# szpiech/garlic

Measured on AMD Instinct MI355X. Metric: LOD-windows/sec (SNPs x inds / winsize), higher is better.
Workload: dtype f64

## Files before the change

garlic_amd/csrc/garlic_hip.hip:

```cpp
#include "../../include/garlic_hip.h"
#include "lod_kernels.hpp"
#include "variant_kernels.hpp"
#include "ld_kernels.hpp"
#include "tgls_ring_kernel.hpp"
#include "wlod_strip_kernel.hpp"
#include "wlod_small_kernel.hpp"
#include "coverage_kernel.hpp"
#include "roh_segments_kernel.hpp"
#include "feed_kernel.hpp"

#include <algorithm>
#include <chrono>
#include <functional>
#include <mutex>
#include <queue>
#include <cmath>
#include <cstdarg>
#include <cstdio>
#include <cstdlib>
#include <cstring>
#include <string>
#include <thread>
#include <unordered_map>
#include <vector>
// ... 1083 lines not shown
    const bool wlod_small = W < WLOD_R;
    if (wlod_shape_ok && use_gl && (rc = ensure_gl_terms(p, true, M, mu))) return rc;
    const bool wlod_gl = wlod_shape_ok && use_gl && p->glterms_valid && p->glterms_scaled;
    bool wlod_fast = (wlod_shape_ok && !use_gl) || wlod_gl;
    if (wlod_fast && !wlod_gl && sizeof(double) * (size_t)(W + TILE) * 4 + 16 > 150 * 1024) wlod_fast = false;
    if (wlod_fast && !wlod_gl && (rc = ensure_score_rows(p, error, M, mu, W))) return rc;
    if (mode == MODE_WLOD && !wlod_fast && (rc = ensure_rld(p))) return rc;
    const bool wlod_stream = wlod_fast && wlod_small && !p->cov_pending.bits && !getenv("GARLIC_WLOD_SMALL_TILES");
    if (p->cov_pending.bits && mode == MODE_WLOD && !wlod_fast) return GARLIC_INTERNAL_NO_BITS;
    if (wlod_stream && (rc = ensure_rld(p))) return rc;
    if (mode == MODE_WLOD && use_gl && p->gl_cont && !wlod_fast && (rc = ensure_gl_terms(p))) return rc;
    const size_t wlod_rows = wlod_gl ? 0 : sizeof(double) * (size_t)(W + TILE) * 4;
    const size_t wlod_patch = sizeof(double) * (size_t)WAVE * WT_PITCH;
    const bool wlod_use_patch = wlod_rows + 16 + wlod_patch <= 160 * 1024 / 8 && !getenv("GARLIC_WLOD_NO_PATCH");
    const bool wlod_gl_ring = wlod_gl && !wlod_small && (ind_begin & (WAVE - 1)) == 0 && !getenv("GARLIC_WLOD_GL_NO_RING");
    const bool ring_patch = !getenv("GARLIC_WLOD_GL_NO_PATCH");
    const int strip_waves = (W + 15 - 16 * WS_WAVES <= 16 || getenv("GARLIC_WLOD_STRIP_NARROW_ONLY")) ? WS_WAVES : WS_WAVES_WIDE;
    const bool wlod_gl_strip = wlod_gl_ring && W + 15 - 16 * strip_waves <= 16 && !getenv("GARLIC_WLOD_GL_NO_STRIP");
    const bool strip_now = wlod_gl_strip;
    const size_t wlod_lds = wlod_gl_ring ? WLOD_GL_RING_OFF + (size_t)WLOD_WAVES * GARLIC_WLOD_GL_RING_ROWS * WAVE * 8
                                   : wlod_rows + 16 + (wlod_use_patch ? wlod_patch : 0);

    const Layout Lhost = make_layout(p, pitch_align, ind_count);
    const int32_t pitch_align_host = pitch_align;
    if (where == GARLIC_HOST) pitch_align = std::max(pitch_align, 32);
    Layout L = make_layout(p, pitch_align, ind_count, thin_step);
    for (int c = 0; c < p->nchr; c++)
        if (3 * L.pitch[c] * 8 + 512 >= (int64_t)1 << 32)
            return fail(GARLIC_ERR_INVALID, "chromosome %d too long for 32-bit row offsets", c);

    const bool feed_kernel = thin_step > 0;
    uint64_t blocks_hash = 0;
    if (blocks) {
        blocks_hash = 0xCBF29CE484222325ull;
        for (uint8_t b : *blocks) blocks_hash = (blocks_hash ^ (b ? 1u : 2u)) * 0x100000001B3ull;
        blocks_hash |= 1;
    }
    const bool reuse = p->plan.valid && p->plan.blocks_hash == blocks_hash && p->plan.mode == (int)mode && p->plan.W == W &&
                       p->plan.max_gap == max_gap && p->plan.ind_begin == ind_begin &&
                       p->plan.ind_count == ind_count && p->plan.pitch_align == pitch_align &&
                       p->plan.wlod_fast == wlod_fast && p->plan.thin_step == thin_step && p->plan.wlod_strip == wlod_gl_strip &&
                       p->plan.feed_kernel == feed_kernel;
    const int nblk = (ind_count + WAVE - 1) / WAVE;
    std::vector<Run> runs;
    std::vector<FillItem> fill;
    std::vector<ChainItem> items;
    std::vector<FeedItem> feed_items;
    std::vector<ChrDev> chrs;
    int64_t n_valid = p->plan.n_valid;
    size_t n_items = p->plan.n_items, n_fill = p->plan.n_fill, n_feed_items = p->plan.n_feed_items;
    int64_t n_runs = p->plan.n_runs;
    if (!reuse) {
        plan_runs(p, W, runs, fill, n_valid);
        std::vector<int> order(runs.size());
        for (size_t i = 0; i < runs.size(); i++) order[i] = (int)i;
        std::stable_sort(order.begin(), order.end(), [&](int x, int y) {
            return (runs[x].b - runs[x].a) > (runs[y].b - runs[y].a);
        });
        items.reserve(runs.size() * nblk);
        for (size_t i = 0; i < order.size(); i++) {
            const Run &r = runs[order[i]];
            for (int k = 0; k < nblk; k++)
                if (!blocks || (*blocks)[(size_t)k]) items.push_back(ChainItem{r.chr, r.a, r.b, k * WAVE});
        }
        if (feed_kernel) {
            std::vector<int32_t> col0(runs.size());
            for (size_t i = 0; i < runs.size(); i++) {
                const int32_t s = (runs[i].a + thin_step - 1) / thin_step;
                col0[i] = (int64_t)s * thin_step <= runs[i].b ? s : -1;
            }
            build_feed_items(runs, order, blocks, nblk, col0, feed_items);
            n_feed_items = feed_items.size();
            if ((rc = p->d_feed_items.reserve(std::max<size_t>(n_feed_items, 1)))) return rc;
        }
        chrs.resize(p->nchr);
        for (int c = 0; c < p->nchr; c++)
            chrs[c] = ChrDev{p->chr_off[c], L.base[c], L.pitch[c], p->chr_nloci[c],
                             (pitch_align >= 2 && 64 * L.pitch[c] * 8 + 512 < ((int64_t)1 << 32)) ? 1 : 0};
        n_items = items.size();
        n_fill = fill.size();
        n_runs = (int64_t)runs.size();
        if ((rc = p->d_chrs.reserve(chrs.size()))) return rc;
        if ((rc = p->d_items.reserve(std::max<size_t>(n_items, 1)))) return rc;
        if ((rc = p->d_fill.reserve(std::max<size_t>(n_fill, 1)))) return rc;
        if (!p->d_counter.p) {
            if ((rc = p->d_counter.reserve(8))) return rc;
            HIP_TRY(hipMemsetAsync(p->d_counter.p, 0, 8 * sizeof(int32_t), ctx->stream));
        }
        p->plan.valid = false;
    }
    std::vector<uint8_t> valid;
    std::vector<int2> tiles, segs;
    if (wlod_fast && !reuse) {
        valid.assign((size_t)p->nloci, 0);
        for (const Run &r : runs)
            memset(valid.data() + p->chr_off[r.chr] + r.a, 1, (size_t)(r.b - r.a + 1));
        for (int c = 0; c < p->nchr; c++)
            for (int s0 = 0; s0 < p->chr_nloci[c]; s0 += TILE) tiles.push_back(make_int2(c, s0));
        p->plan.n_tiles = (int32_t)tiles.size();
        for (int c = 0; c < p->nchr; c++)
            for (int s0 = 0; s0 < p->chr_nloci[c]; s0 += WSM_T) segs.push_back(make_int2(c, s0));
        p->plan.n_segs = (int32_t)segs.size();
        if ((rc = p->d_valid.reserve(valid.size()))) return rc;
        if ((rc = p->d_tiles.reserve(tiles.size())) || (rc = p->d_segs.reserve(segs.size()))) return rc;
    }
    std::vector<WlodStrip> strips;
    if (wlod_gl_strip && !reuse) {
        int64_t total_groups = 0;
        for (int c = 0; c < p->nchr; c++) total_groups += (p->chr_nloci[c] + WLOD_R - 1) / WLOD_R;
        const int64_t pairs = (nblk + 1) / 2;
        int64_t per = total_groups * pairs / 8192;
        per = std::min<int64_t>(256, std::max<int64_t>(64, per)) & ~(int64_t)1;
        if (const char *e = getenv("GARLIC_WLOD_STRIP_GROUPS")) per = std::max<int64_t>(1, atol(e));
        for (int c = 0; c < p->nchr; c++) {
            const int ng = (p->chr_nloci[c] + WLOD_R - 1) / WLOD_R;
            for (int g0 = 0; g0 < ng; g0 += (int)per)
                strips.push_back(WlodStrip{c, g0 * WLOD_R, std::min<int>((int)per, ng - g0), 0});
        }
        p->plan.n_strips = (int32_t)strips.size();
        if ((rc = p->d_strips.reserve(strips.size()))) return rc;
    }
    int workers = ctx->n_cu;
    if (const char *e = getenv("GARLIC_WORKERS")) workers = std::max(1, atoi(e));
    workers = std::min<int>(workers, (int)n_items);

    double *d_out = out;
    if (where == GARLIC_HOST) {
        if (p->d_out.cap < (size_t)L.total && mode == MODE_LOD && thin_step == 0 && !p->placing &&
            (size_t)L.total * sizeof(double) >= ((size_t)1 << 30) && !getenv("GARLIC_NO_PLACEMENT")) {
            p->placing = true;
            void *best = nullptr;
            rc = garlic_panel_alloc_scores(p, pitch_align, ind_count, W, error, max_gap, 0, &best, nullptr);
            p->placing = false;
            if (rc) return rc;
            p->d_out.adopt(ctx, best, (size_t)L.total);
            return launch_lod(p, mode, W, error, max_gap, M, mu, ind_begin, ind_count, pitch_align_host, out, where, thin_step, blocks);
        }
        if ((rc = p->d_out.reserve(ctx, (size_t)L.total))) return rc;
        d_out = p->d_out.p;
    }
    const bool aligned16 = (pitch_align % 2 == 0) && ((reinterpret_cast<uintptr_t>(d_out) & 15) == 0);

    auto enqueue = [&]() -> int {
    HIP_TRY(hipEventRecord(ctx->ev_begin, ctx->stream));
    if (!reuse) {
        HIP_TRY(hipMemcpyAsync(p->d_chrs.p, chrs.data(), sizeof(ChrDev) * chrs.size(),
                               hipMemcpyHostToDevice, ctx->stream));
        if (n_items)
            HIP_TRY(hipMemcpyAsync(p->d_items.p, items.data(), sizeof(ChainItem) * n_items,
                                   hipMemcpyHostToDevice, ctx->stream));
        if (feed_kernel && n_feed_items)
            HIP_TRY(hipMemcpyAsync(p->d_feed_items.p, feed_items.data(), sizeof(FeedItem) * n_feed_items,
                                   hipMemcpyHostToDevice, ctx->stream));
        if (n_fill)
            HIP_TRY(hipMemcpyAsync(p->d_fill.p, fill.data(), sizeof(FillItem) * n_fill,
                                   hipMemcpyHostToDevice, ctx->stream));
        if (wlod_fast) {
            HIP_TRY(hipMemcpyAsync(p->d_valid.p, valid.data(), valid.size(), hipMemcpyHostToDevice,
                                   ctx->stream));
            HIP_TRY(hipMemcpyAsync(p->d_tiles.p, tiles.data(), sizeof(int2) * tiles.size(),
                                   hipMemcpyHostToDevice, ctx->stream));
            HIP_TRY(hipMemcpyAsync(p->d_segs.p, segs.data(), sizeof(int2) * segs.size(),
                                   hipMemcpyHostToDevice, ctx->stream));
            if (!strips.empty())
                HIP_TRY(hipMemcpyAsync(p->d_strips.p, strips.data(), sizeof(WlodStrip) * strips.size(),
                                       hipMemcpyHostToDevice, ctx->stream));
        }
    }
    if (thin_step > 0) {
        hipLaunchKernelGGL(fill_value_kernel, dim3(1024), dim3(256), 0, ctx->stream, d_out, L.total, MISSING_D);
    } else if (n_fill && !wlod_fast && !cov_bits) {
        dim3 grid((unsigned)n_fill, (unsigned)((ind_count + FILL_ROWS - 1) / FILL_ROWS));
        hipLaunchKernelGGL(fill_missing_kernel, grid, dim3(256), 0, ctx->stream, p->d_fill.p,
                           p->d_chrs.p, ind_count, d_out);
    }
    if (n_items && (!reuse || mode != MODE_LOD)) HIP_TRY(hipMemsetAsync(p->d_counter.p, 0, 2 * sizeof(int32_t), ctx->stream));
    p->stats_slot = (int)(ctx->n_calls % garlic_ctx::HIST);
    HIP_TRY(hipEventRecord(ctx->hist0[p->stats_slot], ctx->stream));
    if (wlod_fast) {
        const bool two_blocks = !wlod_gl && !wlod_small && !getenv("GARLIC_WLOD_ONE_BLOCK");
        const int per_wg = two_blocks ? WLOD2_BLOCKS : WLOD_WAVES;
        const int nquad = (nblk + per_wg - 1) / per_wg;
        WlodArgs a{p->d_valid.p, p->d_chrs.p, p->d_tiles.p, p->nwordrows, p->nchr, ind_begin, ind_count, W, nquad,
                   (uint32_t)((int64_t)p->plan.n_tiles * nquad), ((wlod_gl_ring ? ring_patch : wlod_use_patch) ? 1 : 0) | (getenv("GARLIC_WLOD_NO_PF") ? 2 : 0),
                   (int64_t)(GOFF + p->nloci + GPAD_BACK), wlod_gl_ring ? 1 : 0, p->cov_pending, nullptr, nullptr};
        const uint32_t *a_packed = p->d_packed.p;
        const double *a_wtab = wlod_gl ? p->d_glterms.p : p->d_wtab.p, *a_skew = p->d_skew.p + SKEW_FRONT;
        const unsigned wl_grid = (a.n_work + 7u) / 8u * 8u;
        const dim3 wl_block(WLOD_WAVES * WAVE);
        if (wlod_lds > 48 * 1024 && two_blocks) {
            const void *fn = aligned16 ? (const void *)wlod_tile2_kernel<WLOD_R, true> : (const void *)wlod_tile2_kernel<WLOD_R, false>;
            HIP_TRY(hipFuncSetAttribute(fn, hipFuncAttributeMaxDynamicSharedMemorySize, (int)wlod_lds));
        } else if (wlod_lds > 48 * 1024) {
            const void *fn = wlod_gl ? (aligned16 ? (const void *)wlod_tile_gl_kernel<WLOD_R, true>
                                                  : (const void *)wlod_tile_gl_kernel<WLOD_R, false>)
                                     : (aligned16 ? (const void *)wlod_tile_kernel<WLOD_R, true>
                                                  : (const void *)wlod_tile_kernel<WLOD_R, false>);
            HIP_TRY(hipFuncSetAttribute(fn, hipFuncAttributeMaxDynamicSharedMemorySize, (int)wlod_lds));
        }
        if (wlod_stream && aligned16) {
            const int nquad8 = (nblk + WLOD2_BLOCKS - 1) / WLOD2_BLOCKS;
            WlodArgs as = a;
            as.tiles = p->d_segs.p;
            as.nquad = nquad8;
            as.n_work = (uint32_t)((int64_t)p->plan.n_segs * nquad8);
            as.use_patch = 1;
            const void *fn = wlod_gl ? wlod_stream_small_gl_fn(W) : wlod_stream_small_fn(W);
            const size_t lds = wlod_small_lds_bytes(W);
            if (lds > 48 * 1024) HIP_TRY(hipFuncSetAttribute(fn, hipFuncAttributeMaxDynamicSharedMemorySize, (int)lds));
            const double *a_rld = p->d_rld.p;
            void *kargs[] = {(void *)&a_packed, (void *)&a_wtab, (void *)&a_rld, (void *)&d_out, (void *)&as};
            HIP_TRY(hipLaunchKernel(fn, dim3((as.n_work + 7u) / 8u * 8u), wl_block, kargs, lds, ctx->stream));
        } else if (wlod_small) {
            const void *fn = wlod_gl ? (aligned16 ? (const void *)wlod_tile_small_gl_kernel<WLOD_R, true>
                                                  : (const void *)wlod_tile_small_gl_kernel<WLOD_R, false>)
                                     : (aligned16 ? (const void *)wlod_tile_small_kernel<WLOD_R, true>
                                                  : (const void *)wlod_tile_small_kernel<WLOD_R, false>);
            void *kargs[] = {(void *)&a_packed, (void *)&a_wtab, (void *)&a_skew, (void *)&d_out, (void *)&a};
            HIP_TRY(hipLaunchKernel(fn, dim3(wl_grid), wl_block, kargs, wlod_lds, ctx->stream));
        } else if (strip_now) {
            const int n_pairs = (nblk + 1) / 2;
            WlodStripArgs sa{p->d_valid.p, p->d_chrs.p, p->d_strips.p, p->d_glterms.p, a_skew, d_out,
                             (int64_t)(GOFF + p->nloci + GPAD_BACK), ind_begin, ind_count, W, strip_waves, n_pairs,
                             ring_patch ? 1 : 0, (uint32_t)((int64_t)p->plan.n_strips * n_pairs), p->d_counter.p + 3, p->cov_pending};
// ... 2 lines not shown
            const bool wide = strip_waves == WS_WAVES_WIDE;
            bool three = !wide && aligned16 && !sa.cov.bits && !getenv("GARLIC_WLOD_STRIP_TWO_PER_CU");
            for (int k = 0; three && k < p->nchr; k++) three = L.pitch[k] * 8 < ((int64_t)1 << 32);
            const void *fn = three ? (const void *)wlod_strip_gl3_kernel
                             : wide ? (aligned16 ? (const void *)wlod_strip_gl_kernel<true, WS_WAVES_WIDE>
                                                 : (const void *)wlod_strip_gl_kernel<false, WS_WAVES_WIDE>)
                                    : (aligned16 ? (const void *)wlod_strip_gl_kernel<true, WS_WAVES>
                                                 : (const void *)wlod_strip_gl_kernel<false, WS_WAVES>);
            const uint32_t strip_lds = three ? WF_LDS_BYTES : WS_LDS_BYTES;
            HIP_TRY(hipFuncSetAttribute(fn, hipFuncAttributeMaxDynamicSharedMemorySize, (int)strip_lds));
            void *kargs[] = {(void *)&sa};
            HIP_TRY(hipLaunchKernel(fn, dim3(grid), dim3((strip_waves + 1) * WAVE), kargs, strip_lds, ctx->stream));
            if (getenv("GARLIC_WLOD_STRIP_FORCE_RERUN")) HIP_TRY(hipMemsetAsync(p->d_counter.p + 3, 1, sizeof(int32_t), ctx->stream));
            WlodArgs ar = a;
            ar.run_if = p->d_counter.p + 3;
            ar.rerun_count = p->d_counter.p + 4;
            if (aligned16)
                hipLaunchKernelGGL((wlod_tile_glring_kernel<WLOD_R, true>), dim3(wl_grid), wl_block, wlod_lds, ctx->stream,
                                   a_packed, a_wtab, a_skew, d_out, ar);
            else
                hipLaunchKernelGGL((wlod_tile_glring_kernel<WLOD_R, false>), dim3(wl_grid), wl_block, wlod_lds, ctx->stream,
                                   a_packed, a_wtab, a_skew, d_out, ar);
        } else if (wlod_gl_ring && aligned16)
            hipLaunchKernelGGL((wlod_tile_glring_kernel<WLOD_R, true>), dim3(wl_grid), wl_block, wlod_lds, ctx->stream,
                               a_packed, a_wtab, a_skew, d_out, a);
        else if (wlod_gl_ring)
            hipLaunchKernelGGL((wlod_tile_glring_kernel<WLOD_R, false>), dim3(wl_grid), wl_block, wlod_lds, ctx->stream,
                               a_packed, a_wtab, a_skew, d_out, a);
        else if (wlod_gl && aligned16)
            hipLaunchKernelGGL((wlod_tile_gl_kernel<WLOD_R, true>), dim3(wl_grid), wl_block, wlod_lds, ctx->stream,
                               a_packed, a_wtab, a_skew, d_out, a);
        else if (wlod_gl)
            hipLaunchKernelGGL((wlod_tile_gl_kernel<WLOD_R, false>), dim3(wl_grid), wl_block, wlod_lds, ctx->stream,
                               a_packed, a_wtab, a_skew, d_out, a);
        else if (two_blocks && aligned16)
            hipLaunchKernelGGL((wlod_tile2_kernel<WLOD_R, true>), dim3(wl_grid), wl_block, wlod_lds, ctx->stream,
                               a_packed, a_wtab, a_skew, d_out, a);
        else if (two_blocks)
            hipLaunchKernelGGL((wlod_tile2_kernel<WLOD_R, false>), dim3(wl_grid), wl_block, wlod_lds, ctx->stream,
                               a_packed, a_wtab, a_skew, d_out, a);
        else if (aligned16)
            hipLaunchKernelGGL((wlod_tile_kernel<WLOD_R, true>), dim3(wl_grid), wl_block, wlod_lds, ctx->stream,
                               a_packed, a_wtab, a_skew, d_out, a);
        else
            hipLaunchKernelGGL((wlod_tile_kernel<WLOD_R, false>), dim3(wl_grid), wl_block, wlod_lds, ctx->stream,
                               a_packed, a_wtab, a_skew, d_out, a);
    } else if (n_items && exact) {
        VariantArgs a{p->d_packed.p, p->d_tab.p,  p->d_tabgl.p, p->d_codes.p, p->d_decay.p, p->d_rld.p,
                      p->d_items.p,  p->d_chrs.p, d_out,        p->nind_pad,  p->nwordrows, ind_begin,    ind_count,
                      W,             (int32_t)p->gl_values.size(), use_gl ? 1 : 0,
                      (use_gl && p->gl_cont) ? p->d_glterms.p : nullptr, (int64_t)(GOFF + p->nloci + GPAD_BACK)};
        hipLaunchKernelGGL(lod_chain_exact_kernel, dim3((unsigned)n_items), dim3(WAVE), 0, ctx->stream, a, (int)n_items);
    } else if (n_items && mode == MODE_LOD) {
        ChainArgs a{p->d_packed.p, p->d_tab.p, p->d_items.p,     p->d_chrs.p,     d_out, p->nind_pad, p->nwordrows,
                    ind_begin,     ind_count,  W,               (int32_t)n_items, p->d_counter.p, nullptr};
        DevBuf<int64_t> d_trace;
        const char *trace_path = getenv("GARLIC_TRACE");
        if (trace_path && !(feed_kernel && n_feed_items) && d_trace.reserve(4 * n_items) == GARLIC_OK) {
            (void)hipMemsetAsync(d_trace.p, 0, sizeof(int64_t) * 4 * n_items, ctx->stream);
            a.trace = d_trace.p;
        }
        if (feed_kernel && n_feed_items) {
            FeedArgs f{p->d_packed.p, p->d_tab.p, p->d_feed_items.p, p->d_chrs.p, d_out, nullptr, p->nwordrows, ind_begin, ind_count, W,
                       (int32_t)n_feed_items, thin_step, getenv("GARLIC_FEED_NO_ASM") ? 0 : 1, p->d_counter.p, nullptr};
            DevBuf<int64_t> d_ftrace;
            const char *ftrace_path = getenv("GARLIC_TRACE");
            if (ftrace_path && d_ftrace.reserve(8 * n_feed_items) == GARLIC_OK) {
                (void)hipMemsetAsync(d_ftrace.p, 0, sizeof(int64_t) * 8 * n_feed_items, ctx->stream);
                f.trace = d_ftrace.p;
            }
            const void *fn = (const void *)lod_feed_kernel;
            int grid = (int)std::min<size_t>(n_feed_items, (size_t)ctx->n_cu * std::max(1, p->plan.feed_per_cu));
            if (!reuse && (rc = feed_grid(ctx, feed_items, &grid, &p->plan.feed_per_cu))) return rc;
            void *kargs[] = {(void *)&f};
            HIP_TRY(hipLaunchKernel(fn, dim3((unsigned)grid), dim3(FEED_G * WAVE), kargs, 0, ctx->stream));
            if (f.trace) {
                std::vector<int64_t> tr(8 * n_feed_items);
                (void)hipMemcpyAsync(tr.data(), d_ftrace.p, sizeof(int64_t) * tr.size(), hipMemcpyDeviceToHost, ctx->stream);
                (void)hipStreamSynchronize(ctx->stream);
                if (FILE *fo = fopen(ftrace_path, "w")) {
                    for (size_t i = 0; i < n_feed_items; i++) {
                        fprintf(fo, "%zu", i);
                        for (int q = 0; q < 8; q++) fprintf(fo, " %lld", (long long)tr[8 * i + q]);
                        fprintf(fo, "\n");
                    }
                    fclose(fo);
                }
                d_ftrace.release();
            }
        } else if (aligned16)
            hipLaunchKernelGGL((lod_chain_kernel<true>), dim3((unsigned)workers), dim3(CHAIN_THREADS), 0,
                               ctx->stream, a);
        else
            hipLaunchKernelGGL((lod_chain_kernel<false>), dim3((unsigned)workers), dim3(CHAIN_THREADS), 0,
                               ctx->stream, a);
        if (a.trace) {
            std::vector<int64_t> tr(4 * n_items);
            (void)hipMemcpyAsync(tr.data(), d_trace.p, sizeof(int64_t) * tr.size(), hipMemcpyDeviceToHost, ctx->stream);
            (void)hipStreamSynchronize(ctx->stream);
            if (FILE *f = fopen(trace_path, "w")) {
                for (size_t i = 0; i < n_items; i++)
                    fprintf(f, "%zu %lld %lld %lld %lld %d\n", i, (long long)tr[4 * i], (long long)tr[4 * i + 1],
                            (long long)tr[4 * i + 2], (long long)tr[4 * i + 3], 0);
                fclose(f);
            }
            d_trace.release();
        }
    } else if (n_items) {
        VariantArgs a{p->d_packed.p, p->d_tab.p,  p->d_tabgl.p, p->d_codes.p, p->d_decay.p, p->d_rld.p,
                      p->d_items.p,  p->d_chrs.p, d_out,        p->nind_pad,  p->nwordrows, ind_begin,    ind_count,
                      W,             (int32_t)p->gl_values.size(), use_gl ? 1 : 0,
                      (use_gl && p->gl_cont) ? p->d_glterms.p : nullptr, (int64_t)(GOFF + p->nloci + GPAD_BACK)};
        if (mode == MODE_LOD_GL && p->glterms_valid && !p->glterms_scaled && (ind_begin & (WAVE - 1)) == 0 &&
            !getenv("GARLIC_TGLS_NO_RING")) {
            TglsArgs t{p->d_glterms.p, (int64_t)(GOFF + p->nloci + GPAD_BACK), p->d_items.p, p->d_chrs.p, d_out,
                       ind_begin, ind_count, W, (int32_t)n_items, p->d_counter.p, p->cov_pending};
            if (p->cov_pending.bits) p->cov_written = true;
            hipLaunchKernelGGL(lod_chain_ring_kernel, dim3((unsigned)workers), dim3(TG_THREADS), 0, ctx->stream, t);
        } else if (cov_bits) {
            return GARLIC_INTERNAL_NO_BITS;
        } else if (mode == MODE_LOD_GL && p->glterms_valid && !p->glterms_scaled) {
            hipLaunchKernelGGL(lod_chain_terms_kernel, dim3((unsigned)n_items), dim3(2 * WAVE), 0, ctx->stream, a,
                               (int)n_items, (int64_t)(GOFF + p->nloci + GPAD_BACK), p->d_glterms.p);
        } else if (mode == MODE_LOD_GL) {
            hipLaunchKernelGGL(lod_chain_gl_kernel, dim3((unsigned)((n_items + GL_WAVES - 1) / GL_WAVES)),
                               dim3(GL_WAVES * WAVE), 0, ctx->stream, a, (int)n_items);
        } else {
            const int ring = W + TILE;
            const size_t lds = sizeof(double) * ((size_t)ring * WAVE + ((W + 1) & ~1) + (size_t)WAVE * TPITCH);
            if (lds > 160 * 1024)
                return fail(GARLIC_ERR_INVALID, "wLOD with winsize %d: this build supports 2..240 and 16..4096", W);
            HIP_TRY(hipFuncSetAttribute(reinterpret_cast<const void *>(wlod_kernel),
                                        hipFuncAttributeMaxDynamicSharedMemorySize, (int)lds));
            hipLaunchKernelGGL(wlod_kernel, dim3((unsigned)n_items), dim3(WAVE), lds, ctx->stream, a,
                               ring);
        }
    }
    HIP_TRY(hipEventRecord(ctx->hist1[ctx->n_calls % garlic_ctx::HIST], ctx->stream));
    ctx->n_calls++;
    HIP_TRY(hipGetLastError());
    return GARLIC_OK;
    };
    if ((rc = enqueue())) return rc;
    p->last_chain_kind = exact ? 2 : 0;
    if (exact_possible && !exact && n_items) {
        int32_t found = 0;
        HIP_TRY(hipMemsetAsync(p->d_counter.p + 2, 0, sizeof(int32_t), ctx->stream));
        hipLaunchKernelGGL(sentinel_scan_kernel, dim3((unsigned)n_items), dim3(256), 0, ctx->stream, p->d_items.p, p->d_chrs.p,
                           d_out, ind_count, p->d_counter.p + 2);
        HIP_TRY(hipMemcpyAsync(&found, p->d_counter.p + 2, sizeof(int32_t), hipMemcpyDeviceToHost, ctx->stream));
        HIP_TRY(hipStreamSynchronize(ctx->stream));
        p->last_chain_kind = found ? 2 : 1;
        if (found) {
            exact = true;
            if ((rc = enqueue())) return rc;
        }
// ... 1988 lines not shown
```

garlic_amd/csrc/lod_kernels.hpp:

```cpp
#pragma once
#include <hip/hip_runtime.h>
#include <stdint.h>

#include "chain_loop_gfx950.inc"

namespace garlic {

constexpr int WAVE = 64;
constexpr int TILE = 32;
constexpr int TPITCH = 34;
constexpr int GOFF = 32;
constexpr int GPAD_CHAIN = 32 * GARLIC_CHAIN_NSLOT + 48 * GARLIC_CHAIN_CHROWS + 64;
constexpr int GPAD_BACK = GPAD_CHAIN > 4160 ? GPAD_CHAIN : 4160;
constexpr double MISSING_D = -9999.0;

struct ChrDev {
    int64_t loc_base;
    int64_t out_base;
    int64_t out_pitch;
    int32_t nloci;
    int32_t fast;
};

struct ChainItem {
// ... 149 lines not shown

__global__ void __launch_bounds__(SEG_BLOCK)
seg_compact_kernel(const int32_t *pos, const int64_t *chr_off, const int32_t *cs,
                   const int32_t *ce, int nchr, int64_t nloci, int32_t max_gap,
                   const int32_t *block_offsets, int64_t *boundaries)
{
    __shared__ int wsum[SEG_BLOCK / WAVE];
    __shared__ int running;
    if (threadIdx.x == 0) running = block_offsets[blockIdx.x];
    int64_t base = (int64_t)blockIdx.x * SEG_BLOCK * SEG_ITEMS;
    __syncthreads();
    for (int k = 0; k < SEG_ITEMS; k++) {
        int64_t G = base + (int64_t)k * SEG_BLOCK + threadIdx.x;
        int f = boundary_flag(pos, chr_off, cs, ce, nchr, nloci, max_gap, G);
        int inc = wave_inclusive_scan(f);
        if ((threadIdx.x & 63) == 63) wsum[threadIdx.x >> 6] = inc;
        __syncthreads();
        int woff = 0;
        for (int w = 0; w < (int)(threadIdx.x >> 6); w++) woff += wsum[w];
        int start = running;
        if (f) boundaries[start + woff + inc - 1] = G;
        __syncthreads();
        if (threadIdx.x == SEG_BLOCK - 1) running = start + woff + inc;
        __syncthreads();
    }
}

constexpr int FILL_ROWS = 16;
__global__ void __launch_bounds__(256)
fill_missing_kernel(const FillItem *items, const ChrDev *chrs, int32_t nind, double *out)
{
    FillItem it = items[blockIdx.x];
    ChrDev c = chrs[it.chr];
    int wave = threadIdx.x >> 6, lane = threadIdx.x & 63;
    int row0 = blockIdx.y * FILL_ROWS;
    for (int r = row0 + wave; r < row0 + FILL_ROWS && r < nind; r += 4) {
        double *row = out + c.out_base + (int64_t)r * c.out_pitch;
        for (int l = it.lo + lane; l < it.hi; l += WAVE) row[l] = MISSING_D;
    }
}

struct ChainArgs {
    const uint32_t *packed;
    const double *tab;
    const ChainItem *items;
    const ChrDev *chrs;
    double *out;
    int64_t nind_pad;
    int64_t nwordrows;
    int32_t ind_begin;
    int32_t ind_count;
    int32_t winsize;
    int32_t n_items;
    int32_t *next_item;
    int64_t *trace;
};

constexpr uint32_t SLOT_BYTES = 3072;
constexpr uint32_t SL_LW1 = 0, SL_LW2 = 256, SL_TW1 = 512, SL_TW2 = 768;
constexpr uint32_t SL_LTAB = 1024, SL_TTAB = 2048;
constexpr uint32_t LDS_ITEM = 3072;
constexpr uint32_t LDS_TILE = GARLIC_CHAIN_LDS_TILE0;
constexpr uint32_t LDS_BYTES = GARLIC_CHAIN_LDS_TOTAL;
constexpr int CHAIN_THREADS = 256;

struct Streams {
    int64_t lead_w, trail_w;
    const double *lead_tab, *trail_tab;
    int sh_lead, sh_trail;
};

__device__ __forceinline__ void advance(Streams &st)
{
    st.lead_w += 2; st.trail_w += 2;
    st.lead_tab += 4 * TILE; st.trail_tab += 4 * TILE;
}

__device__ __forceinline__ void fill_regs(unsigned char *smem, const Streams &st,
                                          const uint32_t *gcol, int lane)
{
    const uint32_t l1 = gcol[(st.lead_w + 1) * WAVE], l2 = gcol[(st.lead_w + 2) * WAVE];
    const uint32_t t1 = gcol[(st.trail_w + 1) * WAVE], t2 = gcol[(st.trail_w + 2) * WAVE];
    const double2 tl = reinterpret_cast<const double2 *>(st.lead_tab)[lane];
    const double2 tt = reinterpret_cast<const double2 *>(st.trail_tab)[lane];
    *reinterpret_cast<uint32_t *>(smem + SL_LW1 + lane * 4) = l1;
    *reinterpret_cast<uint32_t *>(smem + SL_LW2 + lane * 4) = l2;
    *reinterpret_cast<uint32_t *>(smem + SL_TW1 + lane * 4) = t1;
    *reinterpret_cast<uint32_t *>(smem + SL_TW2 + lane * 4) = t2;
    *reinterpret_cast<double2 *>(smem + SL_LTAB + lane * 16) = tl;
    *reinterpret_cast<double2 *>(smem + SL_TTAB + lane * 16) = tt;
}

struct TileBits {
    uint32_t lead_lo, lead_hi, trail_lo, trail_hi;
};

template <int SLOT>
__device__ __forceinline__ TileBits tile_consume(const unsigned char *smem, uint32_t &lc,
                                                 uint32_t &tc, const Streams &st, int lane)
{
    const unsigned char *slot = smem + SLOT * SLOT_BYTES;
    const uint32_t l1 = *reinterpret_cast<const uint32_t *>(slot + SL_LW1 + lane * 4);
    const uint32_t l2 = *reinterpret_cast<const uint32_t *>(slot + SL_LW2 + lane * 4);
    const uint32_t t1 = *reinterpret_cast<const uint32_t *>(slot + SL_TW1 + lane * 4);
    const uint32_t t2 = *reinterpret_cast<const uint32_t *>(slot + SL_TW2 + lane * 4);
    TileBits tb;
    tb.lead_lo = __builtin_amdgcn_alignbit(l1, lc, st.sh_lead);
    tb.lead_hi = __builtin_amdgcn_alignbit(l2, l1, st.sh_lead);
    tb.trail_lo = __builtin_amdgcn_alignbit(t1, tc, st.sh_trail);
    tb.trail_hi = __builtin_amdgcn_alignbit(t2, t1, st.sh_trail);
    lc = l2;
    tc = t2;
    return tb;
}

template <bool EDGE, int SLOT>
__device__ __forceinline__ void tile_steps(const unsigned char *smem, unsigned char *tile,
                                           double &acc, const TileBits &tb, int s0, int a, int b,
                                           int lane)
{
    const unsigned char *slot = smem + SLOT * SLOT_BYTES;
    const uint32_t tile_lane = (uint32_t)lane * (TPITCH * 8);
#pragma unroll
    for (int j = 0; j < TILE; j++) {
        const uint32_t lw = (j < 16) ? tb.lead_lo : tb.lead_hi;
        const uint32_t tw = (j < 16) ? tb.trail_lo : tb.trail_hi;
        const uint32_t g1 = (lw >> (2 * (j & 15))) & 3u;
        const uint32_t g0 = (tw >> (2 * (j & 15))) & 3u;
        double t_in = *reinterpret_cast<const double *>(slot + SL_LTAB + j * 32 + g1 * 8);
        double t_out = *reinterpret_cast<const double *>(slot + SL_TTAB + j * 32 + g0 * 8);
        if (EDGE) {
            const int s = s0 + j;
            if (!(s > a && s <= b)) t_out = 0.0;
            if (!(s >= a && s <= b)) t_in = 0.0;
        }
        acc = (acc - t_out) + t_in;
        *reinterpret_cast<double *>(tile + tile_lane + j * 8) = acc;
    }
}

template <bool EDGE, bool ALIGNED16>
__device__ __forceinline__ void tile_store(const unsigned char *tile, int s0, int a, int b, int lane,
                                           int rows_valid, double *out_tile, int64_t pitch)
{
    const int rsub = lane >> 4, csub = lane & 15;
#pragma unroll
    for (int q = 0; q < WAVE / 4; q++) {
        const int qe = (4 * q < rows_valid) ? q : 0;
        const int re = min(rsub, rows_valid - 1 - 4 * qe);
        const double2 v = *reinterpret_cast<const double2 *>(
            tile + (uint32_t)(4 * qe + re) * (TPITCH * 8) + csub * 16);
        char *base = reinterpret_cast<char *>(out_tile + (int64_t)(4 * qe) * pitch);
        const uint32_t off = (uint32_t)re * (uint32_t)(pitch * 8) + (uint32_t)csub * 16u;
        double *dst = reinterpret_cast<double *>(base + off);
        if (EDGE) {
            const int s = s0 + 2 * csub;
            if (s >= a && s <= b) dst[0] = v.x;
            if (s + 1 >= a && s + 1 <= b) dst[1] = v.y;
        } else if (!ALIGNED16) {
            dst[0] = v.x;
            dst[1] = v.y;
        } else {
            *reinterpret_cast<double2 *>(dst) = v;
        }
    }
}

__global__ void __launch_bounds__(256) fill_value_kernel(double *dst, int64_t n, double value)
{
    for (int64_t i = (int64_t)blockIdx.x * blockDim.x + threadIdx.x; i < n; i += (int64_t)gridDim.x * blockDim.x)
        dst[i] = value;
}

template <bool ALIGNED16>
__global__ void __launch_bounds__(CHAIN_THREADS)
lod_chain_kernel(ChainArgs p)
{
    __shared__ __attribute__((aligned(16))) unsigned char smem[LDS_BYTES];
    unsigned char *tile = smem + LDS_TILE;
    const int lane = threadIdx.x & (WAVE - 1);
    const int wave = __builtin_amdgcn_readfirstlane(threadIdx.x >> 6);
    for (;;) {
    if (threadIdx.x == 0)
        *reinterpret_cast<int *>(smem + LDS_ITEM) = atomicAdd(p.next_item, 1);
    __syncthreads();
    const int item_idx =
        __builtin_amdgcn_readfirstlane(*reinterpret_cast<const int *>(smem + LDS_ITEM));
    __syncthreads();
    if (item_idx >= p.n_items) {
        if (threadIdx.x == 0) {
            __threadfence();
            if (atomicAdd(p.next_item + 1, 1) == (int)gridDim.x - 1) {
                p.next_item[0] = 0;
                p.next_item[1] = 0;
            }
        }
        return;
    }
    if (p.trace && threadIdx.x == 0) {
        p.trace[4 * item_idx + 0] = blockIdx.x;
        p.trace[4 * item_idx + 1] = wall_clock64();
    }
    const ChainItem it = p.items[item_idx];
    const ChrDev c = p.chrs[it.chr];
    const int W = p.winsize;
    const int a = it.a, b = it.b;
    const int rows_valid = min(WAVE, p.ind_count - it.ind0);
    const int64_t col0 = (int64_t)p.ind_begin + it.ind0;
    const uint32_t *gcol = p.packed + packed_index(0, col0 + lane, p.nwordrows);
    const int64_t Gbase = c.loc_base + GOFF;

    double acc = 0.0;
    if (wave == 0) {
        int l = a;
        const int lend = a + W - 1;
        while (l < lend) {
            const int64_t G = Gbase + l;
            const int sh = 2 * (int)(G & 15);
            const uint32_t *wp = gcol + (G >> 4) * WAVE;
            uint32_t wd[5];
#pragma unroll
            for (int q = 0; q < 5; q++) wd[q] = wp[q * WAVE];
            uint32_t al[4];
#pragma unroll
            for (int q = 0; q < 4; q++) al[q] = __builtin_amdgcn_alignbit(wd[q + 1], wd[q], sh);
            const int n = min(64, lend - l);
            double t[64];
#pragma unroll
            for (int q = 0; q < 64; q++) {
                const uint32_t g = (al[q >> 4] >> (2 * (q & 15))) & 3u;
                t[q] = p.tab[(G + min(q, n - 1)) * 4 + ((q < n) ? g : 3u)];
            }
#pragma unroll
            for (int q = 0; q < 64; q++) acc += (q < n) ? t[q] : 0.0;
            l += n;
        }
    }

    int s0 = a & ~(TILE - 1);
    Streams st;
    {
        const int64_t Glead = Gbase + s0 + W - 1;
        const int64_t Gtrail = Gbase + s0 - 1;
        st.sh_lead = 2 * (int)(Glead & 15);
        st.sh_trail = 2 * (int)(Gtrail & 15);
        st.lead_w = Glead >> 4;
        st.trail_w = Gtrail >> 4;
        st.lead_tab = p.tab + Glead * 4;
        st.trail_tab = p.tab + Gtrail * 4;
    }
    double *const out_row = p.out + c.out_base + (int64_t)it.ind0 * c.out_pitch;
    double *out_tile = out_row + s0;
    const int64_t pitch = c.out_pitch;

    for (int phase = 0; phase < 2; phase++) {
        const int last = (phase == 0) ? s0 : b;
        while (s0 <= last && s0 <= b) {
            if (wave == 0) {
                uint32_t lc = gcol[st.lead_w * WAVE];
                uint32_t tc = gcol[st.trail_w * WAVE];
                fill_regs(smem, st, gcol, lane);
                const TileBits tb = tile_consume<0>(smem, lc, tc, st, lane);
                tile_steps<true, 0>(smem, tile, acc, tb, s0, a, b, lane);
                tile_store<true, ALIGNED16>(tile, s0, a, b, lane, rows_valid, out_tile, pitch);
            }
            advance(st);
            s0 += TILE;
            out_tile += TILE;
        }
        if (phase == 1 || !ALIGNED16 || !c.fast || (col0 & 63) != 0) continue;
        if (st.lead_w - st.trail_w > GARLIC_CHAIN_MAX_DW) continue;

        int ntiles = (b + 1 - s0) / TILE;
        if (ntiles >= 2) {
            uint32_t lc = gcol[st.lead_w * WAVE];
            uint32_t tc = gcol[st.trail_w * WAVE];
            const int64_t chunk0 = st.trail_w / GARLIC_CHAIN_CHROWS;
            const int64_t chunkI = (st.lead_w + 2 * GARLIC_CHAIN_NSLOT) / GARLIC_CHAIN_CHROWS + 1;
            const uint32_t *pchunk =
                p.packed + packed_index(GARLIC_CHAIN_CHROWS * chunk0, col0, p.nwordrows);
            const uint32_t wmask = GARLIC_CHAIN_WROWS - 1;
            if (p.trace && threadIdx.x == 0) p.trace[4 * item_idx + 2] = wall_clock64();
            const uint32_t a_nchunk0 = (uint32_t)(chunkI - chunk0 + 1) * (GARLIC_CHAIN_CHROWS / 4);
            const uint32_t a_roff0 = (uint32_t)((GARLIC_CHAIN_CHROWS * chunk0) & wmask) * 256u;
            const uint32_t a_laddr0 = (uint32_t)(st.lead_w & wmask) * 256u;
            const uint32_t a_taddr0 = (uint32_t)(st.trail_w & wmask) * 256u;
            if (wave == 0) {
                uint32_t tin[4], tout[4];
#pragma unroll
                for (int q = 0; q < 4; q++) {
                    const uint32_t bb = 4u * (uint32_t)lane + (uint32_t)q;
                    const uint32_t sp = (bb & 3u) | (((bb >> 2) & 3u) << 8) | (((bb >> 4) & 3u) << 16) | (((bb >> 6) & 3u) << 24);
                    tin[q] = sp << 4;
                    tout[q] = sp << 6;
                }
                *reinterpret_cast<uint4 *>(smem + GARLIC_CHAIN_SPREAD_IN + lane * 16) = make_uint4(tin[0], tin[1], tin[2], tin[3]);
                *reinterpret_cast<uint4 *>(smem + GARLIC_CHAIN_SPREAD_OUT + lane * 16) = make_uint4(tout[0], tout[1], tout[2], tout[3]);
            }
            {
                asm volatile(GARLIC_CHAIN_LOOP_ASM
                             : [acc] "+v"(acc)
                             : [wave] "s"(wave), [lane] "v"(lane), [lc] "v"(lc), [tc] "v"(tc),
                               [pchunk] "s"(pchunk), [nchunk0] "s"(a_nchunk0), [roff0] "s"(a_roff0),
                               [laddr0] "s"(a_laddr0), [taddr0] "s"(a_taddr0),
                               [pltab] "s"(st.lead_tab), [pttab] "s"(st.trail_tab), [out] "s"(out_tile),
                               [ntiles] "s"(ntiles), [shl] "s"(st.sh_lead), [sht] "s"(st.sh_trail),
                               [pitch8] "s"((uint32_t)(pitch * 8)), [rows] "s"(rows_valid)
                             : GARLIC_CHAIN_LOOP_CLOBBERS);
            }
            st.lead_w += 2 * ntiles;
            st.trail_w += 2 * ntiles;
            st.lead_tab += (int64_t)(4 * TILE) * ntiles;
            st.trail_tab += (int64_t)(4 * TILE) * ntiles;
            s0 += ntiles * TILE;
            out_tile += (int64_t)ntiles * TILE;
            __syncthreads();
        }
    }
    if (p.trace && threadIdx.x == 0) p.trace[4 * item_idx + 3] = wall_clock64();
    }
}

}
```

Baseline: 7.285 billion.

## Fold missing-fill into chain kernel and prefetch next work item

```diff
diff --git a/garlic_amd/csrc/garlic_hip.hip b/garlic_amd/csrc/garlic_hip.hip
--- a/garlic_amd/csrc/garlic_hip.hip
+++ b/garlic_amd/csrc/garlic_hip.hip
@@ -1159,6 +1159,13 @@
     int64_t n_runs = p->plan.n_runs;
     if (!reuse) {
         plan_runs(p, W, runs, fill, n_valid);
+        {
+            std::vector<FillItem> pieces;
+            for (const FillItem &f : fill)
+                for (int32_t lo = f.lo; lo < f.hi; lo += FILL_PIECE)
+                    pieces.push_back(FillItem{f.chr, lo, std::min(f.hi, lo + FILL_PIECE), 0});
+            fill.swap(pieces);
+        }
         std::vector<int> order(runs.size());
         for (size_t i = 0; i < runs.size(); i++) order[i] = (int)i;
         std::stable_sort(order.begin(), order.end(), [&](int x, int y) {
@@ -1227,9 +1234,9 @@
         p->plan.n_strips = (int32_t)strips.size();
         if ((rc = p->d_strips.reserve(strips.size()))) return rc;
     }
-    int workers = ctx->n_cu;
-    if (const char *e = getenv("GARLIC_WORKERS")) workers = std::max(1, atoi(e));
-    workers = std::min<int>(workers, (int)n_items);
+    int workers_max = ctx->n_cu;
+    if (const char *e = getenv("GARLIC_WORKERS")) workers_max = std::max(1, atoi(e));
+    const int workers = std::min<int>(workers_max, (int)n_items);
 
     double *d_out = out;
     if (where == GARLIC_HOST) {
@@ -1249,6 +1256,8 @@
     const bool aligned16 = (pitch_align % 2 == 0) && ((reinterpret_cast<uintptr_t>(d_out) & 15) == 0);
 
     auto enqueue = [&]() -> int {
+    const bool fill_in_chain = n_items && mode == MODE_LOD && !exact && !feed_kernel;
+    const int64_t n_fill_work = fill_in_chain ? (int64_t)n_fill * nblk : 0;
     HIP_TRY(hipEventRecord(ctx->ev_begin, ctx->stream));
     if (!reuse) {
         HIP_TRY(hipMemcpyAsync(p->d_chrs.p, chrs.data(), sizeof(ChrDev) * chrs.size(),
@@ -1276,7 +1285,7 @@
     }
     if (thin_step > 0) {
         hipLaunchKernelGGL(fill_value_kernel, dim3(1024), dim3(256), 0, ctx->stream, d_out, L.total, MISSING_D);
-    } else if (n_fill && !wlod_fast && !cov_bits) {
+    } else if (n_fill && !wlod_fast && !cov_bits && !fill_in_chain) {
         dim3 grid((unsigned)n_fill, (unsigned)((ind_count + FILL_ROWS - 1) / FILL_ROWS));
         hipLaunchKernelGGL(fill_missing_kernel, grid, dim3(256), 0, ctx->stream, p->d_fill.p,
                            p->d_chrs.p, ind_count, d_out);
@@ -1385,12 +1394,15 @@
                       (use_gl && p->gl_cont) ? p->d_glterms.p : nullptr, (int64_t)(GOFF + p->nloci + GPAD_BACK)};
         hipLaunchKernelGGL(lod_chain_exact_kernel, dim3((unsigned)n_items), dim3(WAVE), 0, ctx->stream, a, (int)n_items);
     } else if (n_items && mode == MODE_LOD) {
-        ChainArgs a{p->d_packed.p, p->d_tab.p, p->d_items.p,     p->d_chrs.p,     d_out, p->nind_pad, p->nwordrows,
-                    ind_begin,     ind_count,  W,               (int32_t)n_items, p->d_counter.p, nullptr};
+        ChainArgs a{p->d_packed.p, p->d_tab.p, p->d_items.p, p->d_chrs.p, d_out, p->nind_pad, p->nwordrows,
+                    ind_begin, ind_count, W, (int32_t)n_items, p->d_fill.p, nblk, (int32_t)n_fill_work, p->d_counter.p,
+                    nullptr};
+        const size_t n_traced = n_items + (size_t)n_fill_work;
+        const int chain_workers = (int)std::min<int64_t>(workers_max, (int64_t)n_traced);
         DevBuf<int64_t> d_trace;
         const char *trace_path = getenv("GARLIC_TRACE");
-        if (trace_path && !(feed_kernel && n_feed_items) && d_trace.reserve(4 * n_items) == GARLIC_OK) {
-            (void)hipMemsetAsync(d_trace.p, 0, sizeof(int64_t) * 4 * n_items, ctx->stream);
+        if (trace_path && !(feed_kernel && n_feed_items) && d_trace.reserve(8 * n_traced) == GARLIC_OK) {
+            (void)hipMemsetAsync(d_trace.p, 0, sizeof(int64_t) * 8 * n_traced, ctx->stream);
             a.trace = d_trace.p;
         }
         if (feed_kernel && n_feed_items) {
@@ -1422,19 +1434,20 @@
                 d_ftrace.release();
             }
         } else if (aligned16)
-            hipLaunchKernelGGL((lod_chain_kernel<true>), dim3((unsigned)workers), dim3(CHAIN_THREADS), 0,
+            hipLaunchKernelGGL((lod_chain_kernel<true>), dim3((unsigned)chain_workers), dim3(CHAIN_THREADS), 0,
                                ctx->stream, a);
         else
-            hipLaunchKernelGGL((lod_chain_kernel<false>), dim3((unsigned)workers), dim3(CHAIN_THREADS), 0,
+            hipLaunchKernelGGL((lod_chain_kernel<false>), dim3((unsigned)chain_workers), dim3(CHAIN_THREADS), 0,
                                ctx->stream, a);
         if (a.trace) {
-            std::vector<int64_t> tr(4 * n_items);
+            std::vector<int64_t> tr(8 * n_traced);
             (void)hipMemcpyAsync(tr.data(), d_trace.p, sizeof(int64_t) * tr.size(), hipMemcpyDeviceToHost, ctx->stream);
             (void)hipStreamSynchronize(ctx->stream);
             if (FILE *f = fopen(trace_path, "w")) {
-                for (size_t i = 0; i < n_items; i++)
-                    fprintf(f, "%zu %lld %lld %lld %lld %d\n", i, (long long)tr[4 * i], (long long)tr[4 * i + 1],
-                            (long long)tr[4 * i + 2], (long long)tr[4 * i + 3], 0);
+                for (size_t i = 0; i < n_traced; i++)
+                    fprintf(f, "%zu %lld %lld %lld %lld %d %lld %lld %lld %lld\n", i, (long long)tr[8 * i], (long long)tr[8 * i + 1],
+                            (long long)tr[8 * i + 2], (long long)tr[8 * i + 3], i < n_items ? 0 : 1, (long long)tr[8 * i + 4],
+                            (long long)tr[8 * i + 5], (long long)tr[8 * i + 6], (long long)tr[8 * i + 7]);
                 fclose(f);
             }
             d_trace.release();
diff --git a/garlic_amd/csrc/lod_kernels.hpp b/garlic_amd/csrc/lod_kernels.hpp
--- a/garlic_amd/csrc/lod_kernels.hpp
+++ b/garlic_amd/csrc/lod_kernels.hpp
@@ -225,6 +225,9 @@
     int32_t ind_count;
     int32_t winsize;
     int32_t n_items;
+    const FillItem *fill;
+    int32_t fill_blocks;
+    int32_t n_fill_work;
     int32_t *next_item;
     int64_t *trace;
 };
@@ -233,6 +236,8 @@
 constexpr uint32_t SL_LW1 = 0, SL_LW2 = 256, SL_TW1 = 512, SL_TW2 = 768;
 constexpr uint32_t SL_LTAB = 1024, SL_TTAB = 2048;
 constexpr uint32_t LDS_ITEM = 3072;
+constexpr uint32_t LDS_NEXT_ITEM = 3088, LDS_NEXT_CHR = 3104;
+constexpr int FILL_PIECE = 256;
 constexpr uint32_t LDS_TILE = GARLIC_CHAIN_LDS_TILE0;
 constexpr uint32_t LDS_BYTES = GARLIC_CHAIN_LDS_TOTAL;
 constexpr int CHAIN_THREADS = 256;
@@ -249,19 +254,41 @@
     st.lead_tab += 4 * TILE; st.trail_tab += 4 * TILE;
 }
 
-__device__ __forceinline__ void fill_regs(unsigned char *smem, const Streams &st,
-                                          const uint32_t *gcol, int lane)
-{
-    const uint32_t l1 = gcol[(st.lead_w + 1) * WAVE], l2 = gcol[(st.lead_w + 2) * WAVE];
-    const uint32_t t1 = gcol[(st.trail_w + 1) * WAVE], t2 = gcol[(st.trail_w + 2) * WAVE];
-    const double2 tl = reinterpret_cast<const double2 *>(st.lead_tab)[lane];
-    const double2 tt = reinterpret_cast<const double2 *>(st.trail_tab)[lane];
-    *reinterpret_cast<uint32_t *>(smem + SL_LW1 + lane * 4) = l1;
-    *reinterpret_cast<uint32_t *>(smem + SL_LW2 + lane * 4) = l2;
-    *reinterpret_cast<uint32_t *>(smem + SL_TW1 + lane * 4) = t1;
-    *reinterpret_cast<uint32_t *>(smem + SL_TW2 + lane * 4) = t2;
-    *reinterpret_cast<double2 *>(smem + SL_LTAB + lane * 16) = tl;
-    *reinterpret_cast<double2 *>(smem + SL_TTAB + lane * 16) = tt;
+struct TileRegs {
+    uint32_t lc, tc;
+    uint32_t l1, l2, t1, t2;
+    double2 tl, tt;
+};
+
+__device__ __forceinline__ TileRegs load_tile_regs(const Streams &st, const uint32_t *gcol, int lane)
+{
+    TileRegs r;
+    r.lc = gcol[st.lead_w * WAVE];
+    r.tc = gcol[st.trail_w * WAVE];
+    r.l1 = gcol[(st.lead_w + 1) * WAVE];
+    r.l2 = gcol[(st.lead_w + 2) * WAVE];
+    r.t1 = gcol[(st.trail_w + 1) * WAVE];
+    r.t2 = gcol[(st.trail_w + 2) * WAVE];
+    r.tl = reinterpret_cast<const double2 *>(st.lead_tab)[lane];
+    r.tt = reinterpret_cast<const double2 *>(st.trail_tab)[lane];
+    return r;
+}
+
+__device__ __forceinline__ void store_tile_regs(unsigned char *smem, const TileRegs &r, int lane)
+{
+    *reinterpret_cast<uint32_t *>(smem + SL_LW1 + lane * 4) = r.l1;
+    *reinterpret_cast<uint32_t *>(smem + SL_LW2 + lane * 4) = r.l2;
+    *reinterpret_cast<uint32_t *>(smem + SL_TW1 + lane * 4) = r.t1;
+    *reinterpret_cast<uint32_t *>(smem + SL_TW2 + lane * 4) = r.t2;
+    *reinterpret_cast<double2 *>(smem + SL_LTAB + lane * 16) = r.tl;
+    *reinterpret_cast<double2 *>(smem + SL_TTAB + lane * 16) = r.tt;
+}
+
+__device__ __forceinline__ void load_sum_words(uint32_t (&wd)[5], const uint32_t *gcol, int64_t G)
+{
+    const uint32_t *wp = gcol + (G >> 4) * WAVE;
+#pragma unroll
+    for (int q = 0; q < 5; q++) wd[q] = wp[q * WAVE];
 }
 
 struct TileBits {
@@ -339,6 +366,38 @@
     }
 }
 
+__device__ __forceinline__ void fill_missing_rows(const ChainArgs &p, int f, int wave, int lane)
+{
+    const FillItem fi = p.fill[f / p.fill_blocks];
+    const ChrDev c = p.chrs[fi.chr];
+    const int r0 = (f % p.fill_blocks) * WAVE;
+    const int r1 = min(r0 + WAVE, p.ind_count);
+    for (int r = r0 + wave; r < r1; r += CHAIN_THREADS / WAVE) {
+        double *row = p.out + c.out_base + (int64_t)r * c.out_pitch;
+        for (int l = fi.lo + lane; l < fi.hi; l += WAVE) __builtin_nontemporal_store(MISSING_D, row + l);
+    }
+}
+
+__device__ __forceinline__ int lds_uniform_i32(const unsigned char *smem, uint32_t off)
+{
+    return __builtin_amdgcn_readfirstlane(*reinterpret_cast<const int *>(smem + off));
+}
+
+__device__ __forceinline__ int64_t lds_uniform_i64(const unsigned char *smem, uint32_t off)
+{
+    const uint32_t lo = (uint32_t)lds_uniform_i32(smem, off), hi = (uint32_t)lds_uniform_i32(smem, off + 4);
+    return (int64_t)(((uint64_t)hi << 32) | lo);
+}
+
+template <typename T>
+__device__ __forceinline__ T *uniform_ptr(T *q)
+{
+    const uint64_t u = reinterpret_cast<uint64_t>(q);
+    const uint32_t lo = (uint32_t)__builtin_amdgcn_readfirstlane((int)(uint32_t)u);
+    const uint32_t hi = (uint32_t)__builtin_amdgcn_readfirstlane((int)(uint32_t)(u >> 32));
+    return reinterpret_cast<T *>(((uint64_t)hi << 32) | lo);
+}
+
 __global__ void __launch_bounds__(256) fill_value_kernel(double *dst, int64_t n, double value)
 {
     for (int64_t i = (int64_t)blockIdx.x * blockDim.x + threadIdx.x; i < n; i += (int64_t)gridDim.x * blockDim.x)
@@ -353,13 +412,36 @@
     unsigned char *tile = smem + LDS_TILE;
     const int lane = threadIdx.x & (WAVE - 1);
     const int wave = __builtin_amdgcn_readfirstlane(threadIdx.x >> 6);
+    bool claimed = false;
     for (;;) {
-    if (threadIdx.x == 0)
+    if (threadIdx.x == 0 && !claimed)
         *reinterpret_cast<int *>(smem + LDS_ITEM) = atomicAdd(p.next_item, 1);
     __syncthreads();
-    const int item_idx =
-        __builtin_amdgcn_readfirstlane(*reinterpret_cast<const int *>(smem + LDS_ITEM));
+    const int item_idx = lds_uniform_i32(smem, LDS_ITEM);
+    ChainItem it;
+    ChrDev c;
+    if (claimed && item_idx < p.n_items) {
+        it.chr = lds_uniform_i32(smem, LDS_NEXT_ITEM + 0);
+        it.a = lds_uniform_i32(smem, LDS_NEXT_ITEM + 4);
+        it.b = lds_uniform_i32(smem, LDS_NEXT_ITEM + 8);
+        it.ind0 = lds_uniform_i32(smem, LDS_NEXT_ITEM + 12);
+        c.loc_base = lds_uniform_i64(smem, LDS_NEXT_CHR + 0);
+        c.out_base = lds_uniform_i64(smem, LDS_NEXT_CHR + 8);
+        c.out_pitch = lds_uniform_i64(smem, LDS_NEXT_CHR + 16);
+        c.nloci = lds_uniform_i32(smem, LDS_NEXT_CHR + 24);
+        c.fast = lds_uniform_i32(smem, LDS_NEXT_CHR + 28);
+    }
     __syncthreads();
+    if (item_idx >= p.n_items && item_idx - p.n_items < p.n_fill_work) {
+        if (p.trace && threadIdx.x == 0) {
+            p.trace[8 * item_idx + 0] = blockIdx.x;
+            p.trace[8 * item_idx + 1] = wall_clock64();
+        }
+        fill_missing_rows(p, item_idx - p.n_items, wave, lane);
+        if (p.trace && threadIdx.x == 0) p.trace[8 * item_idx + 3] = wall_clock64();
+        claimed = false;
+        continue;
+    }
     if (item_idx >= p.n_items) {
         if (threadIdx.x == 0) {
             __threadfence();
@@ -371,44 +453,20 @@
         return;
     }
     if (p.trace && threadIdx.x == 0) {
-        p.trace[4 * item_idx + 0] = blockIdx.x;
-        p.trace[4 * item_idx + 1] = wall_clock64();
-    }
-    const ChainItem it = p.items[item_idx];
-    const ChrDev c = p.chrs[it.chr];
+        p.trace[8 * item_idx + 0] = blockIdx.x;
+        p.trace[8 * item_idx + 1] = wall_clock64();
+    }
+    if (!claimed) {
+        it = p.items[item_idx];
+        c = p.chrs[it.chr];
+    }
+    claimed = false;
     const int W = p.winsize;
     const int a = it.a, b = it.b;
     const int rows_valid = min(WAVE, p.ind_count - it.ind0);
     const int64_t col0 = (int64_t)p.ind_begin + it.ind0;
     const uint32_t *gcol = p.packed + packed_index(0, col0 + lane, p.nwordrows);
     const int64_t Gbase = c.loc_base + GOFF;
-
-    double acc = 0.0;
-    if (wave == 0) {
-        int l = a;
-        const int lend = a + W - 1;
-        while (l < lend) {
-            const int64_t G = Gbase + l;
-            const int sh = 2 * (int)(G & 15);
-            const uint32_t *wp = gcol + (G >> 4) * WAVE;
-            uint32_t wd[5];
-#pragma unroll
-            for (int q = 0; q < 5; q++) wd[q] = wp[q * WAVE];
-            uint32_t al[4];
-#pragma unroll
-            for (int q = 0; q < 4; q++) al[q] = __builtin_amdgcn_alignbit(wd[q + 1], wd[q], sh);
-            const int n = min(64, lend - l);
-            double t[64];
-#pragma unroll
-            for (int q = 0; q < 64; q++) {
-                const uint32_t g = (al[q >> 4] >> (2 * (q & 15))) & 3u;
-                t[q] = p.tab[(G + min(q, n - 1)) * 4 + ((q < n) ? g : 3u)];
-            }
-#pragma unroll
-            for (int q = 0; q < 64; q++) acc += (q < n) ? t[q] : 0.0;
-            l += n;
-        }
-    }
 
     int s0 = a & ~(TILE - 1);
     Streams st;
@@ -422,6 +480,35 @@
         st.lead_tab = p.tab + Glead * 4;
         st.trail_tab = p.tab + Gtrail * 4;
     }
+
+    double acc = 0.0;
+    TileRegs head{};
+    if (wave == 0) {
+        head = load_tile_regs(st, gcol, lane);
+        int l = a;
+        const int lend = a + W - 1;
+        uint32_t wd[5];
+        if (l < lend) load_sum_words(wd, gcol, Gbase + l);
+        while (l < lend) {
+            const int64_t G = Gbase + l;
+            const int sh = 2 * (int)(G & 15);
+            uint32_t al[4];
+#pragma unroll
+            for (int q = 0; q < 4; q++) al[q] = __builtin_amdgcn_alignbit(wd[q + 1], wd[q], sh);
+            const int n = min(64, lend - l);
+            if (l + n < lend) load_sum_words(wd, gcol, G + n);
+            double t[64];
+#pragma unroll
+            for (int q = 0; q < 64; q++) {
+                const uint32_t g = (al[q >> 4] >> (2 * (q & 15))) & 3u;
+                t[q] = p.tab[(G + min(q, n - 1)) * 4 + ((q < n) ? g : 3u)];
+            }
+#pragma unroll
+            for (int q = 0; q < 64; q++) acc += (q < n) ? t[q] : 0.0;
+            l += n;
+        }
+    }
+
     double *const out_row = p.out + c.out_base + (int64_t)it.ind0 * c.out_pitch;
     double *out_tile = out_row + s0;
     const int64_t pitch = c.out_pitch;
@@ -430,9 +517,9 @@
         const int last = (phase == 0) ? s0 : b;
         while (s0 <= last && s0 <= b) {
             if (wave == 0) {
-                uint32_t lc = gcol[st.lead_w * WAVE];
-                uint32_t tc = gcol[st.trail_w * WAVE];
-                fill_regs(smem, st, gcol, lane);
+                const TileRegs r = (phase == 0) ? head : load_tile_regs(st, gcol, lane);
+                uint32_t lc = r.lc, tc = r.tc;
+                store_tile_regs(smem, r, lane);
                 const TileBits tb = tile_consume<0>(smem, lc, tc, st, lane);
                 tile_steps<true, 0>(smem, tile, acc, tb, s0, a, b, lane);
                 tile_store<true, ALIGNED16>(tile, s0, a, b, lane, rows_valid, out_tile, pitch);
@@ -446,14 +533,14 @@
 
         int ntiles = (b + 1 - s0) / TILE;
         if (ntiles >= 2) {
-            uint32_t lc = gcol[st.lead_w * WAVE];
-            uint32_t tc = gcol[st.trail_w * WAVE];
+            const uint32_t lc = (wave == 0) ? head.l2 : gcol[st.lead_w * WAVE];
+            const uint32_t tc = (wave == 0) ? head.t2 : gcol[st.trail_w * WAVE];
             const int64_t chunk0 = st.trail_w / GARLIC_CHAIN_CHROWS;
             const int64_t chunkI = (st.lead_w + 2 * GARLIC_CHAIN_NSLOT) / GARLIC_CHAIN_CHROWS + 1;
             const uint32_t *pchunk =
                 p.packed + packed_index(GARLIC_CHAIN_CHROWS * chunk0, col0, p.nwordrows);
             const uint32_t wmask = GARLIC_CHAIN_WROWS - 1;
-            if (p.trace && threadIdx.x == 0) p.trace[4 * item_idx + 2] = wall_clock64();
+            if (p.trace && threadIdx.x == 0) p.trace[8 * item_idx + 2] = wall_clock64();
             const uint32_t a_nchunk0 = (uint32_t)(chunkI - chunk0 + 1) * (GARLIC_CHAIN_CHROWS / 4);
             const uint32_t a_roff0 = (uint32_t)((GARLIC_CHAIN_CHROWS * chunk0) & wmask) * 256u;
             const uint32_t a_laddr0 = (uint32_t)(st.lead_w & wmask) * 256u;
@@ -476,7 +563,7 @@
                              : [wave] "s"(wave), [lane] "v"(lane), [lc] "v"(lc), [tc] "v"(tc),
                                [pchunk] "s"(pchunk), [nchunk0] "s"(a_nchunk0), [roff0] "s"(a_roff0),
                                [laddr0] "s"(a_laddr0), [taddr0] "s"(a_taddr0),
-                               [pltab] "s"(st.lead_tab), [pttab] "s"(st.trail_tab), [out] "s"(out_tile),
+                               [pltab] "s"(st.lead_tab), [pttab] "s"(st.trail_tab), [out] "s"(uniform_ptr(out_tile)),
                                [ntiles] "s"(ntiles), [shl] "s"(st.sh_lead), [sht] "s"(st.sh_trail),
                                [pitch8] "s"((uint32_t)(pitch * 8)), [rows] "s"(rows_valid)
                              : GARLIC_CHAIN_LOOP_CLOBBERS);
@@ -488,10 +575,33 @@
             s0 += ntiles * TILE;
             out_tile += (int64_t)ntiles * TILE;
             __syncthreads();
-        }
-    }
-    if (p.trace && threadIdx.x == 0) p.trace[4 * item_idx + 3] = wall_clock64();
-    }
-}
-
-}
+            if (threadIdx.x == WAVE) {
+                const int nx = atomicAdd(p.next_item, 1);
+                *reinterpret_cast<int *>(smem + LDS_ITEM) = nx;
+                if (nx < p.n_items) {
+                    const ChainItem ni = p.items[nx];
+                    const ChrDev nc = p.chrs[ni.chr];
+                    *reinterpret_cast<int4 *>(smem + LDS_NEXT_ITEM) = make_int4(ni.chr, ni.a, ni.b, ni.ind0);
+                    *reinterpret_cast<int64_t *>(smem + LDS_NEXT_CHR + 0) = nc.loc_base;
+                    *reinterpret_cast<int64_t *>(smem + LDS_NEXT_CHR + 8) = nc.out_base;
+                    *reinterpret_cast<int64_t *>(smem + LDS_NEXT_CHR + 16) = nc.out_pitch;
+                    *reinterpret_cast<int *>(smem + LDS_NEXT_CHR + 24) = nc.nloci;
+                    *reinterpret_cast<int *>(smem + LDS_NEXT_CHR + 28) = nc.fast;
+                }
+            }
+            claimed = true;
+            if (p.trace && threadIdx.x == 0) {
+                p.trace[8 * item_idx + 4] = wall_clock64();
+                p.trace[8 * item_idx + 5] = (int64_t)ntiles * TILE;
+            }
+        }
+    }
+    if (p.trace && threadIdx.x == 0) {
+        p.trace[8 * item_idx + 3] = wall_clock64();
+        p.trace[8 * item_idx + 6] = rows_valid;
+        p.trace[8 * item_idx + 7] = b - a + 1;
+    }
+    }
+}
+
+}
```

Result: no change. 7.410 billion, median of 6 (+1.7%).
